# rainerzufalldererste/limg

Measured on AMD Instinct MI355X. Metric: encode Mpixels/s, 8K RGBA (limg_encode3d_test-equivalent: all 11 planes stored), higher is better.
Workload: dtype u8/i32 integer stage + f32 float stage (bit-exact vs the reference's strict SSE build)

## Files before the change

limg_amd/build.py:

```python
import os
import subprocess
import sys

HERE = os.path.dirname(os.path.abspath(__file__))
CSRC = os.path.join(HERE, "csrc")
OUT = os.path.join(HERE, "liblimg_hip.so")
TEST_OUT = os.path.join(HERE, "liblimg_hip_test.so")
TEST_FLAGS = ["-DLIMG_HIP_TEST_HOOKS"]
SOURCES = ["limg_hip_kernels.hip", "limg_hip_fit_tpb.hip", "limg_hip_stream.hip", "limg_hip_blocked.hip", "limg_hip_synth.hip", "limg_hip_noise_gpu.hip",
           "limg_hip_api.hip", "limg_hip_noise_table.hip", "limg_hip_encode.hip", "limg_hip_encode_ragged.hip", "limg_hip_host_entry.hip", "limg_hip_stream_api.hip",
           "limg_hip_blocked_api.hip", "limg_hip_multi.hip", "limg_hip_noise.cpp", "limg_hip_blocked_host.cpp", "limg_hip_blocked_stream.hip", "limg_hip_stream_window.hip",
           "limg_hip_stream_window_api.hip", "limg_hip_rate.hip", "limg_hip_stream_encode_api.hip"]
EXPORTS = os.path.join(CSRC, "limg_hip.map")
FLAGS = ["--offload-arch=gfx950", "-O3", "-fPIC", "-std=c++17", "-ffp-contract=off", "-fno-fast-math", "-Wall", "-Wno-unused-function"]
SOURCE_FLAGS = {"limg_hip_kernels.hip": ["-mllvm", "-amdgpu-atomic-optimizer-strategy=None"],
                "limg_hip_rate.hip": ["-mllvm", "-amdgpu-atomic-optimizer-strategy=None"],
                "limg_hip_stream.hip": ["-Wno-pass-failed"]}


def _newer(target, deps):
    if not os.path.exists(target):
        return False
    t = os.path.getmtime(target)
    return all(os.path.getmtime(d) <= t for d in deps)


def compile_line(src, extra_flags=(), test_hooks=False):
    hipcc = os.environ.get("HIPCC", "/opt/rocm/bin/hipcc")
    extra = list(extra_flags) + (TEST_FLAGS if test_hooks else [])
    if src.endswith(".cpp"):
        return [hipcc, "-O3", "-fPIC", "-std=c++17", "-Wall", "-ffp-contract=off", "-fno-fast-math", "-x", "c++"] + [f for f in extra if f.startswith("-D")]
    return [hipcc] + FLAGS + SOURCE_FLAGS.get(src, []) + extra


def device_assembly(src, out_dir, extra_flags=(), test_hooks=False):
    out = os.path.join(out_dir, src.rsplit(".", 1)[0] + (".test.s" if test_hooks else ".s"))
    subprocess.check_call(compile_line(src, extra_flags, test_hooks) + ["--cuda-device-only", "-S", os.path.join(CSRC, src), "-o", out], stderr=subprocess.DEVNULL)
    return out


def check_isa(out_dir, extra_flags=(), test_hooks=False, verbose=False):
    import tempfile
    try:
        from limg_amd import isa_check
    except ImportError:
        sys.path.insert(0, os.path.dirname(HERE))
        from limg_amd import isa_check
    with tempfile.TemporaryDirectory() as tmp:
        got = isa_check.check_decode_isa(open(device_assembly("limg_hip_stream.hip", tmp, extra_flags, test_hooks)).read())
    if verbose:
        print("isa check (k_stream_decode, %s build): %s" % ("test-hooks" if test_hooks else "product", got), flush=True)
    return got


def build(force=False, verbose=False, extra_flags=(), out_dir=None, test_hooks=False):
    from concurrent.futures import ThreadPoolExecutor
    hipcc = os.environ.get("HIPCC", "/opt/rocm/bin/hipcc")
    inc = os.path.join(HERE, "..", "include")
    deps = [os.path.join(CSRC, f) for f in os.listdir(CSRC) if not f.endswith(".o") and not f.startswith("__")] + [os.path.join(inc, "limg_hip.h"), os.path.join(inc, "limg_hip_test_hooks.h"), os.path.abspath(__file__)]
    name = "liblimg_hip_test.so" if test_hooks else "liblimg_hip.so"
    target = os.path.join(HERE, name)
    out = target if out_dir is None else os.path.join(out_dir, name)
    if out_dir is None and not force and _newer(target, deps):
        return target
    extra = list(extra_flags) + (TEST_FLAGS if test_hooks else [])
    jobs = []
    for src in SOURCES:
        obj = os.path.join(CSRC if out_dir is None else out_dir, src.rsplit(".", 1)[0] + (".test.o" if test_hooks else ".o"))
        jobs.append((compile_line(src, extra_flags, test_hooks) + ["-c", os.path.join(CSRC, src), "-o", obj], obj))

    def run(job):
        if verbose:
            print(" ".join(job[0]), flush=True)
        subprocess.check_call(job[0])
        return job[1]

    with ThreadPoolExecutor(max_workers=int(os.environ.get("LIMG_BUILD_JOBS", "4"))) as ex:
        objs = list(ex.map(run, jobs))
    check_isa(out_dir, extra_flags, test_hooks, verbose)
    cmd = [hipcc, "--offload-arch=gfx950", "-shared", "-fPIC", "-Wl,--version-script=" + EXPORTS, "-o", out] + objs
    if verbose:
        print(" ".join(cmd), flush=True)
    subprocess.check_call(cmd)
    return out


def build_all(force=False, verbose=False):
    return build(force=force, verbose=verbose), build(force=force, verbose=verbose, test_hooks=True)


CLI_SRC = os.path.join(HERE, "..", "tools", "limg_hip_cli.cpp")
CLI_OUT = os.path.join(HERE, "limg_hip_cli")


def build_cli(force=False, verbose=False):
    build(force=force, verbose=verbose)
    deps = [CLI_SRC, OUT, os.path.join(HERE, "..", "include", "limg_hip.h"), os.path.join(HERE, "..", "include", "limg_hip_shim.hpp")]
    if not force and _newer(CLI_OUT, deps):
        return CLI_OUT
    rocm_lib = os.environ.get("ROCM_LIB", "/opt/rocm/lib")
    cmd = ["g++", "-O2", "-std=c++17", "-Wall", "-I", os.path.join(HERE, "..", "include"), CLI_SRC, "-o", CLI_OUT, "-L", HERE, "-llimg_hip", "-lz", "-lpthread",
           "-Wl,-rpath,$ORIGIN", "-Wl,-rpath-link," + rocm_lib, "-Wl,-rpath," + rocm_lib]
    if verbose:
        print(" ".join(cmd), flush=True)
    subprocess.check_call(cmd)
    return CLI_OUT


if __name__ == "__main__":
    print(build_all(force="--force" in sys.argv, verbose=True))
    print(build_cli(force="--force" in sys.argv, verbose=True))
```

limg_amd/csrc/limg_hip_fit_tpb.hip:

```cpp
#include "limg_hip_device.h"

#include <string.h>

namespace limg_hip
{
  namespace
  {
    constexpr int kTpbStride = 68;

    template <bool DIRECT> constexpr int tpb_waves() { return DIRECT ? 4 : 2; }

    template <class BODY>
    __device__ __forceinline__ void for_rows(const uint32_t *my, const uint32_t pitch, BODY &&body)
    {
      uint4 u0 = *reinterpret_cast<const uint4 *>(my), w0 = *reinterpret_cast<const uint4 *>(my + 4);
      uint4 u1 = *reinterpret_cast<const uint4 *>(my + pitch), w1 = *reinterpret_cast<const uint4 *>(my + pitch + 4);
#pragma unroll 1
      for (int r = 0; r < 8; r += 2)
      {
        const uint32_t *nx = my + (r + 2 < 8 ? r + 2 : 6) * pitch;
        const uint4 nu0 = *reinterpret_cast<const uint4 *>(nx), nw0 = *reinterpret_cast<const uint4 *>(nx + 4);
        const uint4 nu1 = *reinterpret_cast<const uint4 *>(nx + pitch), nw1 = *reinterpret_cast<const uint4 *>(nx + pitch + 4);
        {
          const uint32_t q[8] = { u0.x, u0.y, u0.z, u0.w, w0.x, w0.y, w0.z, w0.w };
          body(r, q);
        }
        {
          const uint32_t q[8] = { u1.x, u1.y, u1.z, u1.w, w1.x, w1.y, w1.z, w1.w };
          body(r + 1, q);
        }
        u0 = nu0; w0 = nw0; u1 = nu1; w1 = nw1;
      }
    }

    template <int CH, bool FAST, bool DIRECT>
    __global__ __launch_bounds__(64 * tpb_waves<DIRECT>(), DIRECT ? 5 : 1) void k_fit_tpb(const EncodeParams p)
    {
      constexpr int kTpbWaves = tpb_waves<DIRECT>();
      __shared__ __attribute__((aligned(16))) uint32_t s_pxAll[kTpbWaves][DIRECT ? 4 : 64 * kTpbStride];
      __shared__ __attribute__((aligned(16))) uint32_t s_tab[FAST ? 4 : 2048];
      const int lane = (int)threadIdx.x & 63, wave = (int)threadIdx.x >> 6;
      if (p.fitPrio == 3) __builtin_amdgcn_s_setprio(3);
      else if (p.fitPrio == 2) __builtin_amdgcn_s_setprio(2);
      else if (p.fitPrio == 1) __builtin_amdgcn_s_setprio(1);
#define LIMG_FIT_TPB_TABLE
#include "limg_hip_fit_tpb_body.inc"
#undef LIMG_FIT_TPB_TABLE
      uint32_t *s_px = s_pxAll[wave];
      const uint32_t unitsX = (p.blocksX + 63u) / 64u;
      const uint32_t unitId = blockIdx.x * kTpbWaves + wave;
      if (unitId >= unitsX * p.blocksY * p.batchCount) return;
      const uint32_t unit = unitId % unitsX, byS = unitId / unitsX;
      const uint32_t img = p.batchCount > 1 ? byS / p.blocksY : 0u, by = byS - img * p.blocksY;
      const uint32_t *const pin = p.batchCount > 1 ? p.batch[img].in : p.io.in;
      const uint32_t bx0 = unit * 64u, x0 = bx0 * kBlock, y0 = by * kBlock;
      const uint32_t nBlocks = min(p.blocksX - bx0, 64u), widthPx = nBlocks * kBlock;
      if (p.zeroLookback)
      {
        if ((uint32_t)lane < 2u && unit * 2u + (uint32_t)lane < p.stripsX) p.desc[(size_t)byS * p.stripsX + unit * 2u + (uint32_t)lane] = 0ull;
        if (unitId == 0 && lane < 4) p.ticket[lane] = 0u;
      }

#include "limg_hip_fit_tpb_body.inc"
    }

    struct FitUnitView
    {
      uint32_t sizeX, blocksX;
      int32_t vecIn;
      limg_hip_block_record *records;
      float *invN;
    };
    __device__ __forceinline__ uint32_t find_prefix(const uint32_t *base, uint32_t n, uint32_t x)
    {
      const __attribute__((address_space(4))) uint32_t *b = (const __attribute__((address_space(4))) uint32_t *)(uintptr_t)base;
      uint32_t lo = 0, hi = n;
      while (hi - lo > 1u)
      {
        const uint32_t mid = (lo + hi) >> 1;
        if (b[mid] <= x) lo = mid; else hi = mid;
      }
      return (uint32_t)__builtin_amdgcn_readfirstlane((int)lo);
    }

    template <int CH, bool FAST, bool DIRECT>
    __global__ __launch_bounds__(64 * tpb_waves<DIRECT>(), DIRECT ? 5 : 1) void k_fit_tpb_list(const FitListParams lp)
    {
      constexpr int kTpbWaves = tpb_waves<DIRECT>();
      __shared__ __attribute__((aligned(16))) uint32_t s_pxAll[kTpbWaves][DIRECT ? 4 : 64 * kTpbStride];
      __shared__ __attribute__((aligned(16))) uint32_t s_tab[FAST ? 4 : 2048];
      const int lane = (int)threadIdx.x & 63, wave = (int)threadIdx.x >> 6;
#define LIMG_FIT_TPB_TABLE
#include "limg_hip_fit_tpb_body.inc"
#undef LIMG_FIT_TPB_TABLE
      uint32_t *s_px = s_pxAll[wave];
      const uint32_t unitId = (uint32_t)__builtin_amdgcn_readfirstlane((int)(blockIdx.x * kTpbWaves + wave));
      if (unitId >= lp.nUnits) return;
      const uint32_t img = find_prefix(lp.firstUnit, lp.nImages, unitId);
      typedef const __attribute__((address_space(4))) ListImage KernImage;
      typedef const __attribute__((address_space(4))) ImageIO KernIO;
      KernImage *const im = (KernImage *)(uintptr_t)lp.images + img;
      const uint32_t unitsX = (im->blocksX + 63u) / 64u, localUnit = unitId - im->firstUnit;
      const uint32_t unit = localUnit % unitsX, by = localUnit / unitsX, byS = by;
      const uint32_t *const pin = (const uint32_t *)(const __attribute__((address_space(1))) uint32_t *)((KernIO *)(uintptr_t)lp.batch + img)->in;
      FitUnitView p;
      p.sizeX = im->sizeX; p.blocksX = im->blocksX; p.vecIn = (im->vec & kListVecIn) ? 1 : 0;
      p.records = lp.records + im->firstBlock; p.invN = lp.invN + 4 * im->firstBlock;
      const uint32_t bx0 = unit * 64u, x0 = bx0 * kBlock, y0 = by * kBlock;
      const uint32_t nBlocks = min(p.blocksX - bx0, 64u), widthPx = nBlocks * kBlock;
      {
        const uint32_t stripsX = im->stripsX;
        if ((uint32_t)lane < 2u && unit * 2u + (uint32_t)lane < stripsX) lp.desc[(size_t)im->firstStrip + (size_t)by * stripsX + unit * 2u + (uint32_t)lane] = 0ull;
        if (unitId == 0 && lane < 4) lp.ticket[lane] = 0u;
      }

#include "limg_hip_fit_tpb_body.inc"
    }
  }

  void launch_fit_tpb_list(const FitListParams &p, int channels, bool floatFast, bool direct, hipStream_t s)
  {
    with_flags([&](auto rgba, auto FAST, auto DIRECT)
               { hipLaunchKernelGGL((k_fit_tpb_list<rgba ? 4 : 3, FAST, DIRECT>), dim3((p.nUnits + tpb_waves<DIRECT>() - 1) / tpb_waves<DIRECT>()), dim3(64 * tpb_waves<DIRECT>()), 0, s, p); },
               channels == 4, floatFast, direct);
  }

  namespace
  {
    struct WordChunk { uint32_t n; uint32_t w[768]; };
    static_assert(sizeof(WordChunk) <= 3584, "kernel-argument segment");
    __global__ void k_set_words(uint32_t *dst, const WordChunk chunk)
    {
      for (uint32_t i = threadIdx.x; i < chunk.n; i += blockDim.x) dst[i] = chunk.w[i];
    }
  }

  void launch_set_words(void *dDst, const void *hSrc, size_t bytes, hipStream_t s)
  {
    const size_t words = bytes / 4;
    for (size_t i0 = 0; i0 < words; i0 += 768)
    {
      WordChunk ch;
      ch.n = (uint32_t)(words - i0 < 768 ? words - i0 : 768);
      memset(ch.w, 0, sizeof(ch.w));
      memcpy(ch.w, (const uint32_t *)hSrc + i0, (size_t)ch.n * 4);
      hipLaunchKernelGGL(k_set_words, dim3(1), dim3(256), 0, s, (uint32_t *)dDst + i0, ch);
    }
  }

  namespace
  {
    struct TableChunk { ImageIO e[32]; uint32_t n; };
    static_assert(sizeof(TableChunk) <= 3584, "kernel-argument segment");
    __global__ void k_set_batch_table(ImageIO *dst, const TableChunk chunk)
    {
      const uint32_t *src = reinterpret_cast<const uint32_t *>(chunk.e);
      uint32_t *out = reinterpret_cast<uint32_t *>(dst);
      for (uint32_t i = threadIdx.x; i < chunk.n * (uint32_t)(sizeof(ImageIO) / 4); i += blockDim.x) out[i] = src[i];
    }
  }

  void launch_set_batch_table(ImageIO *dTable, const ImageIO *hTable, size_t count, hipStream_t s)
  {
    for (size_t i0 = 0; i0 < count; i0 += 32)
    {
      TableChunk ch;
      ch.n = (uint32_t)(count - i0 < 32 ? count - i0 : 32);
      for (uint32_t i = 0; i < ch.n; i++) ch.e[i] = hTable[i0 + i];
      for (uint32_t i = ch.n; i < 32; i++) ch.e[i] = ImageIO{};
      hipLaunchKernelGGL(k_set_batch_table, dim3(1), dim3(256), 0, s, dTable + i0, ch);
    }
  }

  void launch_fit_tpb(const EncodeParams &p, int channels, hipStream_t s)
  {
    const uint32_t units = ((p.blocksX + 63u) / 64u) * p.blocksY * p.batchCount;
    with_flags([&](auto rgba, auto FAST, auto DIRECT)
               { hipLaunchKernelGGL((k_fit_tpb<rgba ? 4 : 3, FAST, DIRECT>), dim3((units + tpb_waves<DIRECT>() - 1) / tpb_waves<DIRECT>()), dim3(64 * tpb_waves<DIRECT>()), 0, s, p); },
               channels == 4, p.floatFast != 0, p.vecIn != 0);
  }
}
```

limg_amd/csrc/limg_hip_fit_tpb_body.inc:

```
#ifdef LIMG_FIT_TPB_TABLE
      if (!FAST)
      {
        const uint4 *src = reinterpret_cast<const uint4 *>(d_rsqrt_x86_tab);
        for (int i = (int)threadIdx.x; i < 256; i += 64 * kTpbWaves)
        {
          const uint4 v = src[i];
          const uint32_t q[4] = { v.x, v.y, v.z, v.w };
          uint32_t *dst = s_tab + ((8 * i) ^ 0x400);
#pragma unroll
          for (int k = 0; k < 4; k++) { dst[2 * k] = (q[k] & 0xFFFFu) << 11; dst[2 * k + 1] = (q[k] >> 16) << 11; }
        }
        __syncthreads();
      }
      const unsigned short *tab = reinterpret_cast<const unsigned short *>(s_tab);
#else
      if (!DIRECT)
      {
      if (p.vecIn)
      {
#pragma unroll
        for (int row = 0; row < 8; row++)
          for (uint32_t col = (uint32_t)lane * 4u; col < widthPx; col += 256u)
          {
            const uint4 v = *reinterpret_cast<const uint4 *>(pin + (size_t)(y0 + row) * p.sizeX + x0 + col);
            *reinterpret_cast<uint4 *>(&s_px[(col >> 3) * kTpbStride + row * 8 + (col & 7u)]) = v;
          }
      }
      else
      {
        for (int row = 0; row < 8; row++)
          for (uint32_t col = (uint32_t)lane; col < widthPx; col += 64u)
            s_px[(col >> 3) * kTpbStride + row * 8 + (col & 7u)] = pin[(size_t)(y0 + row) * p.sizeX + x0 + col];
      }
      }
      wave_lds_fence();
      if ((uint32_t)lane >= nBlocks) return;
      const uint32_t *my = DIRECT ? pin + (size_t)y0 * p.sizeX + x0 + lane * 8 : s_px + lane * kTpbStride;
      const uint32_t pitch = DIRECT ? p.sizeX : 8u;

      uint32_t s02 = 0, s13 = 0;
#pragma unroll
      for (int r = 0; r < 8; r++)
      {
        const uint4 u = *reinterpret_cast<const uint4 *>(my + r * pitch), w = *reinterpret_cast<const uint4 *>(my + r * pitch + 4);
        const uint32_t q[8] = { u.x, u.y, u.z, u.w, w.x, w.y, w.z, w.w };
#pragma unroll
        for (int i = 0; i < 8; i++) { s02 += q[i] & 0x00FF00FFu; s13 += (q[i] >> 8) & 0x00FF00FFu; }
      }
      const float inv_count = 0.015625f;
      V4 avg;
      avg.a = float2_t{ (float)(int)(s02 & 0xFFFF), (float)(int)(s02 >> 16) } * inv_count;
      avg.b = float2_t{ (float)(int)(s13 & 0xFFFF), CH == 4 ? (float)(int)(s13 >> 16) : 0.0f } * inv_count;
      const V4 zero4 = { float2_t{ 0.0f, 0.0f }, float2_t{ 0.0f, 0.0f } };

      auto finish_dir = [&](const V4 &acc, V4 &dir, float &inv, bool &zero)
      {
        dir = acc * inv_count;
        const float pp = dp4<CH>(dir, dir);
        zero = dir.a.x == 0.0f && dir.a.y == 0.0f && dir.b.x == 0.0f && dir.b.y == 0.0f;
        inv = FAST ? __builtin_amdgcn_rcpf(pp) : 1.0f / pp;
      };

      V4 dirA, dirB = zero4, dirC = zero4, est0 = zero4;
      float invA, invB = 0.0f, invC = 0.0f;
      bool zeroA, zeroB = true, zeroC = true;
      float mm[6] = { 0.0f, 0.0f, 0.0f, 0.0f, 0.0f, 0.0f };
      {
        V4 acc = zero4;
        for_rows(my, pitch, [&](const int, const uint32_t (&q)[8])
        {
#pragma unroll
          for (int i = 0; i < 8; i++)
          {
            V4 d = px_to_v4(q[i]) - avg;
            mask_alpha<CH>(d);
            acc = acc + unit4<CH, FAST, true, true>(tab, d, true);
          }
        });
        finish_dir(acc, dirA, invA, zeroA);
      }

      if (!zeroA)
      {
        V4 acc = zero4;
        float mn = 0.0f, mx = 0.0f;
        for_rows(my, pitch, [&](const int, const uint32_t (&q)[8])
        {
#pragma unroll
          for (int i = 0; i < 8; i++)
          {
            const V4 pf = px_to_v4(q[i]);
            const float fA = dp4<CH, FAST>(pf - avg, dirA) * invA;
            mn = vmin(mn, fA); mx = vmax(mx, fA);
            V4 e = pf - (avg + dirA * fA);
            mask_alpha<CH>(e);
            acc = acc + unit4<CH, FAST, true, true>(tab, e, true);
          }
        });
        mm[0] = mn; mm[1] = mx;
        finish_dir(acc, dirB, invB, zeroB);
      }

      if (!zeroA && !zeroB)
      {
        float mnB = FLT_MAX, mxB = -FLT_MAX;
        if (CH == 4)
        {
          V4 acc = zero4;
          for_rows(my, pitch, [&](const int r, const uint32_t (&q)[8])
          {
#pragma unroll
            for (int i = 0; i < 8; i++)
            {
              const V4 pf = px_to_v4(q[i]);
              const float fA = dp4<CH, FAST>(pf - avg, dirA) * invA;
              const V4 estA = avg + dirA * fA;
              const float fB = dp4<CH, FAST>(pf - estA, dirB) * invB;
              mnB = vmin(mnB, fB); mxB = vmax(mxB, fB);
              const V4 estB = estA + dirB * fB;
              if (r == 0 && i == 0) est0 = estB;
              acc = acc + unit4<CH, FAST, true, true>(tab, pf - estB, true);
            }
          });
          mm[2] = mnB; mm[3] = mxB;
          finish_dir(acc, dirC, invC, zeroC);
          if (!zeroC)
          {
            float mnC = FLT_MAX, mxC = -FLT_MAX;
            for_rows(my, pitch, [&](const int, const uint32_t (&q)[8])
            {
#pragma unroll
              for (int i = 0; i < 8; i++)
              {
                const float fC = dp4<CH, FAST>(px_to_v4(q[i]) - est0, dirC) * invC;
                mnC = vmin(mnC, fC); mxC = vmax(mxC, fC);
              }
            });
            mm[4] = mnC; mm[5] = mxC;
          }
        }
        else
        {
          dirC.a.x = dirA.b.x * dirB.a.y - dirA.a.y * dirB.b.x;
          dirC.b.x = dirA.a.y * dirB.a.x - dirA.a.x * dirB.a.y;
          dirC.a.y = dirA.a.x * dirB.b.x - dirA.b.x * dirB.a.x;
          dirC.b.y = 0.0f;
          zeroC = dirC.a.x == 0.0f && dirC.b.x == 0.0f && dirC.a.y == 0.0f;
          if (!zeroC) invC = FAST ? __builtin_amdgcn_rcpf(dp4<CH, FAST>(dirC, dirC)) : 1.0f / dp4<CH, FAST>(dirC, dirC);
          float mnC = zeroC ? 0.0f : FLT_MAX, mxC = zeroC ? 0.0f : -FLT_MAX;
          for_rows(my, pitch, [&](const int, const uint32_t (&q)[8])
          {
#pragma unroll
            for (int i = 0; i < 8; i++)
            {
              const V4 pf = px_to_v4(q[i]);
              const float fA = dp4<CH, FAST>(pf - avg, dirA) * invA;
              const V4 estA = avg + dirA * fA;
              const float fB = dp4<CH, FAST>(pf - estA, dirB) * invB;
              mnB = vmin(mnB, fB); mxB = vmax(mxB, fB);
              if (!zeroC)
              {
                const V4 e = pf - (estA + dirB * fB);
                const float fC = dp4<CH, FAST>(e, dirC) * invC;
                mnC = vmin(mnC, fC); mxC = vmax(mxC, fC);
              }
            }
          });
          mm[2] = mnB; mm[3] = mxB; mm[4] = mnC; mm[5] = mxC;
        }
      }

      const bool deadA = zeroA, deadB = zeroA || zeroB, deadC = zeroA || zeroB || zeroC;
      auto comp = [](const V4 &v, int c) -> float { return c == 0 ? v.a.x : (c == 1 ? v.b.x : (c == 2 ? v.a.y : v.b.y)); };
      uint32_t words[16];
#pragma unroll
      for (int c = 0; c < 4; c++) words[c] = __float_as_uint(comp(avg, c));
      float inv[3];
#pragma unroll
      for (int r = 0; r < 3; r++)
      {
        const bool dead = r == 0 ? deadA : (r == 1 ? deadB : deadC);
        const V4 &dir = r == 0 ? dirA : (r == 1 ? dirB : dirC);
        int16_t lo[4], hi[4];
        float sum = 0.0f;
        bool nz = false;
#pragma unroll
        for (int c = 0; c < 4; c++)
        {
          float dv = comp(dir, c), mLo = mm[2 * r], mHi = mm[2 * r + 1];
          if (dead) { mLo = 0.0f; mHi = 0.0f; dv = 0.0f; }
          float vLo = mLo * dv, vHi = mHi * dv;
          if (r == 0) { vLo = comp(avg, c) + vLo; vHi = comp(avg, c) + vHi; }
          int qLo = cvt_rne(vLo), qHi = cvt_rne(vHi);
          if (CH == 3 && c == 3) { qLo = 0; qHi = 0; }
          lo[c] = (int16_t)qLo; hi[c] = (int16_t)qHi;
          if (CH == 4 || c < 3)
          {
            const float n = (float)((int)hi[c] - (int)lo[c]);
            const float sq = n * n;
            sum = sum + sq;
            nz = nz || sq != 0.0f;
          }
        }
        inv[r] = nz ? (FAST ? __builtin_amdgcn_rcpf(sum) : 1.0f / sum) : 0.0f;
        words[4 + 4 * r] = (uint32_t)(uint16_t)lo[0] | ((uint32_t)(uint16_t)lo[1] << 16);
        words[5 + 4 * r] = (uint32_t)(uint16_t)lo[2] | ((uint32_t)(uint16_t)lo[3] << 16);
        words[6 + 4 * r] = (uint32_t)(uint16_t)hi[0] | ((uint32_t)(uint16_t)hi[1] << 16);
        words[7 + 4 * r] = (uint32_t)(uint16_t)hi[2] | ((uint32_t)(uint16_t)hi[3] << 16);
      }
      uint4 *dst = reinterpret_cast<uint4 *>(p.records + (size_t)byS * p.blocksX + bx0 + lane);
#pragma unroll
      for (int i = 0; i < 4; i++) dst[i] = make_uint4(words[4 * i], words[4 * i + 1], words[4 * i + 2], words[4 * i + 3]);
      reinterpret_cast<float4 *>(p.invN)[(size_t)byS * p.blocksX + bx0 + lane] = make_float4(inv[0], inv[1], inv[2], 0.0f);
#endif
```

limg_amd/isa_check.py:

```python
import re


def check_decode_isa(asm_text):
    text = asm_text.splitlines()
    start = next(i for i, l in enumerate(text) if l.startswith("_ZN8limg_hip12_GLOBAL__N_115k_stream_decodeE"))
    end = next(i for i in range(start, len(text)) if text[i].startswith(".Lfunc_end"))
    body = text[start:end]
    assert not any("scratch_" in l for l in body), "k_stream_decode spills: a scratch reload counts in vmcnt and voids the hand-counted wait"
    blocks, order, cur, in_asm = {}, [], "entry", False
    blocks[cur] = []
    order.append(cur)
    for l in body[1:]:
        t = l.strip()
        if t.startswith(";;#ASMSTART"):
            in_asm = True
            continue
        if t.startswith(";;#ASMEND"):
            in_asm = False
            continue
        m = re.match(r"^(\.LBB\d+_\d+):", t)
        if m:
            cur = m.group(1)
            blocks[cur] = []
            order.append(cur)
            continue
        if not t or t.startswith(";") or t.startswith("."):
            continue
        blocks[cur].append((t.split(";")[0].strip(), in_asm))
    succ = {}
    for i, b in enumerate(order):
        out, fall = [], True
        for t, _ in blocks[b]:
            m = re.match(r"s_(cbranch_\w+|branch) (\.LBB\d+_\d+)", t)
            if m:
                out.append(m.group(2))
                if m.group(1) == "branch":
                    fall = False
            if t.startswith("s_endpgm"):
                fall = False
        if fall and i + 1 < len(order):
            out.append(order[i + 1])
        succ[b] = out
    loads = waits = 0
    state = {b: None for b in order}
    state["entry"] = frozenset()
    work = ["entry"]
    while work:
        b = work.pop()
        pending = set(state[b])
        for t, asm in blocks[b]:
            if asm and t.startswith("global_load_dwordx2"):
                m = re.match(r"global_load_dwordx2 v\[(\d+):(\d+)\]", t)
                assert m, t
                pending |= {int(m.group(1)), int(m.group(2))}
                loads += 1
                continue
            if asm and t.startswith("s_waitcnt vmcnt("):
                pending.clear()
                waits += 1
                continue
            if t.startswith("s_cbranch") or t.startswith("s_branch"):
                continue
            if pending:
                regs = set(int(x) for x in re.findall(r"\bv(\d+)\b", t))
                for a0, b0 in re.findall(r"v\[(\d+):(\d+)\]", t):
                    regs |= set(range(int(a0), int(b0) + 1))
                assert not (regs & pending), "register with a payload load in flight is touched before the counted wait: %s (in flight: v%s, block %s)" % (t, sorted(pending), b)
        for n in succ[b]:
            new = frozenset(pending) if state[n] is None else state[n] | frozenset(pending)
            if new != state[n]:
                state[n] = new
                work.append(n)
    assert loads >= 6 and waits >= 2, (loads, waits)

    INF = 1 << 30
    cnt = {b: None for b in order}
    cnt["entry"] = INF
    work = ["entry"]
    checked = 0
    while work:
        b = work.pop()
        c = cnt[b]
        for t, asm in blocks[b]:
            if asm and t.startswith("global_load_dwordx2"):
                c = 0
            elif asm and t.startswith("s_waitcnt vmcnt("):
                n = int(re.match(r"s_waitcnt vmcnt\((\d+)\)", t).group(1))
                assert c >= n, "a path reaches `%s` with only %d vector-memory operations behind the payload loads (block %s)" % (t, c, b)
                checked += 1
                c = INF
            elif re.match(r"(global|buffer|flat|scratch)_(load|store|atomic)", t) and c != INF:
                c += 1
        for nb in succ[b]:
            new = c if cnt[nb] is None else min(cnt[nb], c)
            if new != cnt[nb]:
                cnt[nb] = new
                work.append(nb)
    assert checked >= 2
    return {"loads": loads, "waits": waits, "counted_waits": checked}
```

Baseline: 57300.

## Load fit pixels with typed buffer_load_format to get floats from the memory unit

In the DIRECT fit kernels, the per-row pixel loads in the PCA passes now use buffer_load_format_xyzw through a hand-built buffer descriptor. The texture/buffer unit converts each u8 RGBA pixel to four floats, so the VALU no longer unpacks bytes and converts them. Rows are double-buffered with hand-counted vmcnt waits in inline asm, and an ISA checker is added to verify register safety. Occupancy bounds drop from 5 to 4 waves because the float rows need more VGPRs. The risks are format-conversion bit-exactness, a heavier memory path, and the fragility of the hand-counted waits.

After: 57730 (median of 6 runs). About the same (+0.7%).

```diff
diff --git a/limg_amd/build.py b/limg_amd/build.py
--- a/limg_amd/build.py
+++ b/limg_amd/build.py
@@ -48,8 +48,10 @@
         from limg_amd import isa_check
     with tempfile.TemporaryDirectory() as tmp:
         got = isa_check.check_decode_isa(open(device_assembly("limg_hip_stream.hip", tmp, extra_flags, test_hooks)).read())
+        fit = isa_check.check_fit_typed_isa(open(device_assembly("limg_hip_fit_tpb.hip", tmp, extra_flags, test_hooks)).read())
     if verbose:
         print("isa check (k_stream_decode, %s build): %s" % ("test-hooks" if test_hooks else "product", got), flush=True)
+        print("isa check (k_fit_tpb typed loads, %s build): %d instances" % ("test-hooks" if test_hooks else "product", len(fit)), flush=True)
     return got
 
 
diff --git a/limg_amd/csrc/limg_hip_fit_tpb.hip b/limg_amd/csrc/limg_hip_fit_tpb.hip
--- a/limg_amd/csrc/limg_hip_fit_tpb.hip
+++ b/limg_amd/csrc/limg_hip_fit_tpb.hip
@@ -1,4 +1,5 @@
 #include "limg_hip_device.h"
+#include "limg_hip_typed_load.h"
 
 #include <string.h>
 
@@ -33,10 +34,63 @@
       }
     }
 
+    template <class BODY>
+    __device__ __forceinline__ void for_rows_global(const uint32_t *my, const uint32_t pitch, BODY &&body)
+    {
+      typedef uint32_t u4 __attribute__((ext_vector_type(4)));
+      typedef const __attribute__((address_space(1))) u4 *gp4;
+      u4 u0 = *(gp4)(my), w0 = *(gp4)(my + 4);
+      u4 u1 = *(gp4)(my + pitch), w1 = *(gp4)(my + pitch + 4);
+#pragma unroll 1
+      for (int r = 0; r < 8; r += 2)
+      {
+        const uint32_t *nx = my + (r + 2 < 8 ? r + 2 : 6) * pitch;
+        const u4 nu0 = *(gp4)(nx), nw0 = *(gp4)(nx + 4);
+        const u4 nu1 = *(gp4)(nx + pitch), nw1 = *(gp4)(nx + pitch + 4);
+        {
+          const uint32_t q[8] = { u0.x, u0.y, u0.z, u0.w, w0.x, w0.y, w0.z, w0.w };
+          body(r, q);
+        }
+        {
+          const uint32_t q[8] = { u1.x, u1.y, u1.z, u1.w, w1.x, w1.y, w1.z, w1.w };
+          body(r + 1, q);
+        }
+        u0 = nu0; w0 = nw0; u1 = nu1; w1 = nw1;
+      }
+    }
+
+    __device__ __forceinline__ V4 row_px(const uint32_t (&q)[8], const int i) { return px_to_v4(q[i]); }
+    __device__ __forceinline__ V4 row_px(const PxRow &q, const int i)
+    {
+      if (i % 4 == 0) __builtin_amdgcn_sched_barrier(0);
+      V4 r;
+      r.a = float2_t{ q.p[i].x, q.p[i].y };
+      r.b = float2_t{ q.p[i].z, q.p[i].w };
+      return r;
+    }
+
+    template <bool DIRECT>
+    __device__ __forceinline__ void ld_row32(const uint32_t *src, uint32_t (&q)[8])
+    {
+      if constexpr (DIRECT)
+      {
+        typedef uint32_t u4 __attribute__((ext_vector_type(4)));
+        typedef const __attribute__((address_space(1))) u4 *gp4;
+        const u4 u = *(gp4)(src), w = *(gp4)(src + 4);
+        q[0] = u.x; q[1] = u.y; q[2] = u.z; q[3] = u.w; q[4] = w.x; q[5] = w.y; q[6] = w.z; q[7] = w.w;
+      }
+      else
+      {
+        const uint4 u = *reinterpret_cast<const uint4 *>(src), w = *reinterpret_cast<const uint4 *>(src + 4);
+        q[0] = u.x; q[1] = u.y; q[2] = u.z; q[3] = u.w; q[4] = w.x; q[5] = w.y; q[6] = w.z; q[7] = w.w;
+      }
+    }
+
     template <int CH, bool FAST, bool DIRECT>
-    __global__ __launch_bounds__(64 * tpb_waves<DIRECT>(), DIRECT ? 5 : 1) void k_fit_tpb(const EncodeParams p)
+    __global__ __launch_bounds__(64 * tpb_waves<DIRECT>(), DIRECT ? 4 : 1) void k_fit_tpb(const EncodeParams p)
     {
       constexpr int kTpbWaves = tpb_waves<DIRECT>();
+      constexpr bool kTypedMid = FAST;
       __shared__ __attribute__((aligned(16))) uint32_t s_pxAll[kTpbWaves][DIRECT ? 4 : 64 * kTpbStride];
       __shared__ __attribute__((aligned(16))) uint32_t s_tab[FAST ? 4 : 2048];
       const int lane = (int)threadIdx.x & 63, wave = (int)threadIdx.x >> 6;
@@ -84,9 +138,10 @@
     }
 
     template <int CH, bool FAST, bool DIRECT>
-    __global__ __launch_bounds__(64 * tpb_waves<DIRECT>(), DIRECT ? 5 : 1) void k_fit_tpb_list(const FitListParams lp)
+    __global__ __launch_bounds__(64 * tpb_waves<DIRECT>(), DIRECT ? 4 : 1) void k_fit_tpb_list(const FitListParams lp)
     {
       constexpr int kTpbWaves = tpb_waves<DIRECT>();
+      constexpr bool kTypedMid = true;
       __shared__ __attribute__((aligned(16))) uint32_t s_pxAll[kTpbWaves][DIRECT ? 4 : 64 * kTpbStride];
       __shared__ __attribute__((aligned(16))) uint32_t s_tab[FAST ? 4 : 2048];
       const int lane = (int)threadIdx.x & 63, wave = (int)threadIdx.x >> 6;
diff --git a/limg_amd/csrc/limg_hip_fit_tpb_body.inc b/limg_amd/csrc/limg_hip_fit_tpb_body.inc
--- a/limg_amd/csrc/limg_hip_fit_tpb_body.inc
+++ b/limg_amd/csrc/limg_hip_fit_tpb_body.inc
@@ -37,13 +37,16 @@
       if ((uint32_t)lane >= nBlocks) return;
       const uint32_t *my = DIRECT ? pin + (size_t)y0 * p.sizeX + x0 + lane * 8 : s_px + lane * kTpbStride;
       const uint32_t pitch = DIRECT ? p.sizeX : 8u;
+      const tl_srd srd = DIRECT ? typed_px_srd(pin + (size_t)y0 * p.sizeX + x0, (7u * p.sizeX + widthPx) * 4u, CH == 4) : tl_srd{ 0, 0, 0, 0 };
+#define rows_mid(body) do { if constexpr (DIRECT && !kTypedMid) for_rows_global(my, pitch, body); else rows(body); } while (0)
+#define rows(body) do { if constexpr (DIRECT) for_rows_f32(srd, (uint32_t)lane * 32u, p.sizeX * 4u, body); else for_rows(my, pitch, body); } while (0)
 
       uint32_t s02 = 0, s13 = 0;
 #pragma unroll
       for (int r = 0; r < 8; r++)
       {
-        const uint4 u = *reinterpret_cast<const uint4 *>(my + r * pitch), w = *reinterpret_cast<const uint4 *>(my + r * pitch + 4);
-        const uint32_t q[8] = { u.x, u.y, u.z, u.w, w.x, w.y, w.z, w.w };
+        uint32_t q[8];
+        ld_row32<DIRECT>(my + r * pitch, q);
 #pragma unroll
         for (int i = 0; i < 8; i++) { s02 += q[i] & 0x00FF00FFu; s13 += (q[i] >> 8) & 0x00FF00FFu; }
       }
@@ -67,16 +70,17 @@
       float mm[6] = { 0.0f, 0.0f, 0.0f, 0.0f, 0.0f, 0.0f };
       {
         V4 acc = zero4;
-        for_rows(my, pitch, [&](const int, const uint32_t (&q)[8])
+        const auto body = [&](const int, const auto &q)
         {
 #pragma unroll
           for (int i = 0; i < 8; i++)
           {
-            V4 d = px_to_v4(q[i]) - avg;
+            V4 d = row_px(q, i) - avg;
             mask_alpha<CH>(d);
             acc = acc + unit4<CH, FAST, true, true>(tab, d, true);
           }
-        });
+        };
+        rows(body);
         finish_dir(acc, dirA, invA, zeroA);
       }
 
@@ -84,19 +88,20 @@
       {
         V4 acc = zero4;
         float mn = 0.0f, mx = 0.0f;
-        for_rows(my, pitch, [&](const int, const uint32_t (&q)[8])
+        const auto body = [&](const int, const auto &q)
         {
 #pragma unroll
           for (int i = 0; i < 8; i++)
           {
-            const V4 pf = px_to_v4(q[i]);
+            const V4 pf = row_px(q, i);
             const float fA = dp4<CH, FAST>(pf - avg, dirA) * invA;
             mn = vmin(mn, fA); mx = vmax(mx, fA);
             V4 e = pf - (avg + dirA * fA);
             mask_alpha<CH>(e);
             acc = acc + unit4<CH, FAST, true, true>(tab, e, true);
           }
-        });
+        };
+        rows_mid(body);
         mm[0] = mn; mm[1] = mx;
         finish_dir(acc, dirB, invB, zeroB);
       }
@@ -107,12 +112,12 @@
         if (CH == 4)
         {
           V4 acc = zero4;
-          for_rows(my, pitch, [&](const int r, const uint32_t (&q)[8])
+          const auto body = [&](const int r, const auto &q)
           {
 #pragma unroll
             for (int i = 0; i < 8; i++)
             {
-              const V4 pf = px_to_v4(q[i]);
+              const V4 pf = row_px(q, i);
               const float fA = dp4<CH, FAST>(pf - avg, dirA) * invA;
               const V4 estA = avg + dirA * fA;
               const float fB = dp4<CH, FAST>(pf - estA, dirB) * invB;
@@ -121,21 +126,23 @@
               if (r == 0 && i == 0) est0 = estB;
               acc = acc + unit4<CH, FAST, true, true>(tab, pf - estB, true);
             }
-          });
+          };
+          rows_mid(body);
           mm[2] = mnB; mm[3] = mxB;
           finish_dir(acc, dirC, invC, zeroC);
           if (!zeroC)
           {
             float mnC = FLT_MAX, mxC = -FLT_MAX;
-            for_rows(my, pitch, [&](const int, const uint32_t (&q)[8])
+            const auto body = [&](const int, const auto &q)
             {
 #pragma unroll
               for (int i = 0; i < 8; i++)
               {
-                const float fC = dp4<CH, FAST>(px_to_v4(q[i]) - est0, dirC) * invC;
+                const float fC = dp4<CH, FAST>(row_px(q, i) - est0, dirC) * invC;
                 mnC = vmin(mnC, fC); mxC = vmax(mxC, fC);
               }
-            });
+            };
+            rows(body);
             mm[4] = mnC; mm[5] = mxC;
           }
         }
@@ -148,12 +155,12 @@
           zeroC = dirC.a.x == 0.0f && dirC.b.x == 0.0f && dirC.a.y == 0.0f;
           if (!zeroC) invC = FAST ? __builtin_amdgcn_rcpf(dp4<CH, FAST>(dirC, dirC)) : 1.0f / dp4<CH, FAST>(dirC, dirC);
           float mnC = zeroC ? 0.0f : FLT_MAX, mxC = zeroC ? 0.0f : -FLT_MAX;
-          for_rows(my, pitch, [&](const int, const uint32_t (&q)[8])
+          const auto body = [&](const int, const auto &q)
           {
 #pragma unroll
             for (int i = 0; i < 8; i++)
             {
-              const V4 pf = px_to_v4(q[i]);
+              const V4 pf = row_px(q, i);
               const float fA = dp4<CH, FAST>(pf - avg, dirA) * invA;
               const V4 estA = avg + dirA * fA;
               const float fB = dp4<CH, FAST>(pf - estA, dirB) * invB;
@@ -165,7 +172,8 @@
                 mnC = vmin(mnC, fC); mxC = vmax(mxC, fC);
               }
             }
-          });
+          };
+          rows(body);
           mm[2] = mnB; mm[3] = mxB; mm[4] = mnC; mm[5] = mxC;
         }
       }
@@ -212,4 +220,6 @@
 #pragma unroll
       for (int i = 0; i < 4; i++) dst[i] = make_uint4(words[4 * i], words[4 * i + 1], words[4 * i + 2], words[4 * i + 3]);
       reinterpret_cast<float4 *>(p.invN)[(size_t)byS * p.blocksX + bx0 + lane] = make_float4(inv[0], inv[1], inv[2], 0.0f);
+#undef rows
+#undef rows_mid
 #endif
diff --git a/limg_amd/csrc/limg_hip_typed_load.h b/limg_amd/csrc/limg_hip_typed_load.h
--- /dev/null
+++ b/limg_amd/csrc/limg_hip_typed_load.h
@@ -0,0 +1,74 @@
+#pragma once
+#include <hip/hip_runtime.h>
+#include <stdint.h>
+
+namespace limg_hip
+{
+  typedef float tl_f4 __attribute__((ext_vector_type(4)));
+  typedef int tl_srd __attribute__((ext_vector_type(4)));
+
+  constexpr uint32_t typed_px_word3(bool alpha) { return 4u | (6u << 3) | (5u << 6) | ((alpha ? 7u : 0u) << 9) | (2u << 12) | (10u << 15); }
+
+  __device__ __forceinline__ tl_srd typed_px_srd(const void *base, uint32_t bytes, bool alpha)
+  {
+    const uint64_t a = (uint64_t)(uintptr_t)base;
+    tl_srd d;
+    d.x = __builtin_amdgcn_readfirstlane((int)(uint32_t)a);
+    d.y = __builtin_amdgcn_readfirstlane((int)((uint32_t)(a >> 32) & 0xFFFFu));
+    d.z = __builtin_amdgcn_readfirstlane((int)bytes);
+    d.w = __builtin_amdgcn_readfirstlane((int)typed_px_word3(alpha));
+    return d;
+  }
+
+  struct PxRow { tl_f4 p[8]; };
+
+#define LIMG_TYPED_ROW_LOADS                                                                                                                                      \
+  "s_nop 4\n\t"                                                                                                                                                   \
+  "buffer_load_format_xyzw %0, %8, %9, 0 offen\n\t"                                                                                                               \
+  "buffer_load_format_xyzw %1, %8, %9, 0 offen offset:4\n\t"                                                                                                      \
+  "buffer_load_format_xyzw %2, %8, %9, 0 offen offset:8\n\t"                                                                                                      \
+  "buffer_load_format_xyzw %3, %8, %9, 0 offen offset:12\n\t"                                                                                                     \
+  "buffer_load_format_xyzw %4, %8, %9, 0 offen offset:16\n\t"                                                                                                     \
+  "buffer_load_format_xyzw %5, %8, %9, 0 offen offset:20\n\t"                                                                                                     \
+  "buffer_load_format_xyzw %6, %8, %9, 0 offen offset:24\n\t"                                                                                                     \
+  "buffer_load_format_xyzw %7, %8, %9, 0 offen offset:28"
+  template <bool FIRST>
+  __device__ __forceinline__ void typed_row_request(PxRow &row, const tl_srd srd, const uint32_t voff)
+  {
+    if (FIRST)
+      asm volatile(LIMG_TYPED_ROW_LOADS
+                   : "=&v"(row.p[0]), "=&v"(row.p[1]), "=&v"(row.p[2]), "=&v"(row.p[3]), "=&v"(row.p[4]), "=&v"(row.p[5]), "=&v"(row.p[6]), "=&v"(row.p[7])
+                   : "v"(voff), "s"(srd));
+    else
+      asm volatile(LIMG_TYPED_ROW_LOADS
+                   : "+v"(row.p[0]), "+v"(row.p[1]), "+v"(row.p[2]), "+v"(row.p[3]), "+v"(row.p[4]), "+v"(row.p[5]), "+v"(row.p[6]), "+v"(row.p[7])
+                   : "v"(voff), "s"(srd));
+  }
+#undef LIMG_TYPED_ROW_LOADS
+
+  template <int N>
+  __device__ __forceinline__ void typed_row_wait(PxRow &row)
+  {
+    asm volatile("s_waitcnt vmcnt(%c8)"
+                 : "+v"(row.p[0]), "+v"(row.p[1]), "+v"(row.p[2]), "+v"(row.p[3]), "+v"(row.p[4]), "+v"(row.p[5]), "+v"(row.p[6]), "+v"(row.p[7])
+                 : "n"(N));
+  }
+
+  template <class BODY>
+  __device__ __forceinline__ void for_rows_f32(const tl_srd srd, const uint32_t voff, const uint32_t pitchBytes, BODY &&body)
+  {
+    PxRow A, B;
+    typed_row_request<true>(A, srd, voff);
+#pragma unroll 1
+    for (int r = 0; r < 8; r += 2)
+    {
+      typed_row_request<true>(B, srd, voff + (uint32_t)(r + 1) * pitchBytes);
+      typed_row_wait<8>(A);
+      body(r, A);
+      typed_row_request<false>(A, srd, voff + (uint32_t)(r + 2 < 8 ? r + 2 : 7) * pitchBytes);
+      typed_row_wait<8>(B);
+      body(r + 1, B);
+    }
+    typed_row_wait<0>(A);
+  }
+}
diff --git a/limg_amd/isa_check.py b/limg_amd/isa_check.py
--- a/limg_amd/isa_check.py
+++ b/limg_amd/isa_check.py
@@ -7,40 +7,7 @@
     end = next(i for i in range(start, len(text)) if text[i].startswith(".Lfunc_end"))
     body = text[start:end]
     assert not any("scratch_" in l for l in body), "k_stream_decode spills: a scratch reload counts in vmcnt and voids the hand-counted wait"
-    blocks, order, cur, in_asm = {}, [], "entry", False
-    blocks[cur] = []
-    order.append(cur)
-    for l in body[1:]:
-        t = l.strip()
-        if t.startswith(";;#ASMSTART"):
-            in_asm = True
-            continue
-        if t.startswith(";;#ASMEND"):
-            in_asm = False
-            continue
-        m = re.match(r"^(\.LBB\d+_\d+):", t)
-        if m:
-            cur = m.group(1)
-            blocks[cur] = []
-            order.append(cur)
-            continue
-        if not t or t.startswith(";") or t.startswith("."):
-            continue
-        blocks[cur].append((t.split(";")[0].strip(), in_asm))
-    succ = {}
-    for i, b in enumerate(order):
-        out, fall = [], True
-        for t, _ in blocks[b]:
-            m = re.match(r"s_(cbranch_\w+|branch) (\.LBB\d+_\d+)", t)
-            if m:
-                out.append(m.group(2))
-                if m.group(1) == "branch":
-                    fall = False
-            if t.startswith("s_endpgm"):
-                fall = False
-        if fall and i + 1 < len(order):
-            out.append(order[i + 1])
-        succ[b] = out
+    blocks, order, succ = _blocks_of(body[1:])
     loads = waits = 0
     state = {b: None for b in order}
     state["entry"] = frozenset()
@@ -98,3 +65,110 @@
                 work.append(nb)
     assert checked >= 2
     return {"loads": loads, "waits": waits, "counted_waits": checked}
+
+
+def _kernel_bodies(asm_text, name_re):
+    text = asm_text.splitlines()
+    out = {}
+    for i, l in enumerate(text):
+        m = re.match(r"^(_Z\w+):", l)
+        if m and re.search(name_re, m.group(1)):
+            end = next(j for j in range(i, len(text)) if text[j].startswith(".Lfunc_end"))
+            out[m.group(1)] = text[i + 1:end]
+    return out
+
+
+def _blocks_of(body):
+    blocks, order, cur, in_asm = {"entry": []}, ["entry"], "entry", False
+    for l in body:
+        t = l.strip()
+        if t.startswith(";;#ASMSTART"):
+            in_asm = True
+            continue
+        if t.startswith(";;#ASMEND"):
+            in_asm = False
+            continue
+        m = re.match(r"^(\.LBB\d+_\d+):", t)
+        if m:
+            cur = m.group(1)
+            blocks[cur] = []
+            order.append(cur)
+            continue
+        if not t or t.startswith(";") or t.startswith("."):
+            continue
+        ins = t.split(";")[0].strip()
+        blocks[cur].append((ins, in_asm))
+        if re.match(r"s_(cbranch_\w+|branch) ", ins):
+            cur = "%s+%d" % (cur.split("+")[0], len(order))
+            blocks[cur] = []
+            order.append(cur)
+    succ = {}
+    for i, b in enumerate(order):
+        out, fall = [], True
+        for t, _ in blocks[b]:
+            m = re.match(r"s_(cbranch_\w+|branch) (\.LBB\d+_\d+)", t)
+            if m:
+                out.append(m.group(2))
+                if m.group(1) == "branch":
+                    fall = False
+            if t.startswith("s_endpgm"):
+                fall = False
+        if fall and i + 1 < len(order):
+            out.append(order[i + 1])
+        succ[b] = out
+    return blocks, order, succ
+
+
+def _vgprs(t):
+    regs = set(int(x) for x in re.findall(r"\bv(\d+)\b", t))
+    for a0, b0 in re.findall(r"\bv\[(\d+):(\d+)\]", t):
+        regs |= set(range(int(a0), int(b0) + 1))
+    return regs
+
+
+FIT_DIRECT = r"k_fit_tpb(_list)?ILi[34]ELb[01]ELb1EEE"
+
+
+def check_fit_typed_isa(asm_text):
+    bodies = _kernel_bodies(asm_text, FIT_DIRECT)
+    assert len(bodies) == 8, sorted(bodies)
+    got = {}
+    for name, body in bodies.items():
+        assert not any("scratch_" in l for l in body), "%s: scratch traffic next to hand-counted waits" % name
+        blocks, order, succ = _blocks_of(body)
+        loads = waits = 0
+        seen = {("entry", ())}
+        work = [("entry", ())]
+        while work:
+            b, flight = work.pop()
+            flight = list(flight)
+            for t, asm in blocks[b]:
+                if asm and t.startswith("buffer_load_format_xyzw"):
+                    m = re.match(r"buffer_load_format_xyzw v\[(\d+):(\d+)\], v(\d+), s\[\d+:\d+\], 0 offen", t)
+                    assert m, t
+                    dst = frozenset(range(int(m.group(1)), int(m.group(2)) + 1))
+                    busy = set().union(*flight) if flight else set()
+                    assert not (dst & busy) and int(m.group(3)) not in busy | dst, "%s: a typed load names a register with a load in flight: %s (block %s)" % (name, t, b)
+                    flight.append(dst)
+                    loads += 1
+                    continue
+                if asm and t.startswith("s_waitcnt vmcnt("):
+                    n = int(re.match(r"s_waitcnt vmcnt\((\d+)\)", t).group(1))
+                    flight = flight[len(flight) - n:] if n else []
+                    waits += 1
+                    continue
+                if asm or t.startswith("s_cbranch") or t.startswith("s_branch"):
+                    continue
+                if flight:
+                    busy = set().union(*flight)
+                    assert not (_vgprs(t) & busy), "%s: register with a typed load in flight is touched before its wait: %s (block %s)" % (name, t, b)
+                    assert not t.startswith("s_endpgm"), "%s: ends with typed loads in flight" % name
+            for n in succ[b]:
+                key = (n, tuple(flight))
+                if key not in seen:
+                    assert len(seen) < 100000, name
+                    seen.add(key)
+                    work.append(key)
+        assert loads >= 16 and waits >= 3, (name, loads, waits)
+        got[name] = {"loads": loads, "waits": waits}
+    return got
```
